# CWBudde/algo-dsp

Measured on AMD Instinct MI355X. Metric: Msamples/sec, overlap-save conv 131072-tap IR @48kHz; achieved HBM GB/s, higher is better.
Workload: dtype f64

## Files before the change

### algo-dsp_amd/csrc/conv_long_kernels.hip

```cpp
#include "conv_long_kernels.hpp"

#include "conv_kernels.hpp"
#include "fft_device.hpp"

namespace adsp {

constexpr int N1 = kLongN1, N2 = kLongN2, W = kLongW;
constexpr int kColThreads = 256;
constexpr int kRowsPerInstr = kColThreads / W;
constexpr int FS = N1 + 1;
using ColPlan = FftPlan<N1, 16>;
constexpr int RV = 8;
using RowPlan = FftPlan<N2, RV>;
static_assert(ColPlan::T * (W / 2) == kColThreads, "a tile's transforms fill the workgroup");
static_assert(N1 % kRowsPerInstr == 0, "whole load rounds");
static_assert(ColPlan::T <= 64 && 64 % ColPlan::T == 0, "a column transform sits inside one wave");

__global__ __launch_bounds__(kColThreads) void k_long_cols_fwd(LongColArgs a) {
  __shared__ double2 lds[(W / 2) * FS];
  __shared__ double2 ltab[TwSplit<N1>::N];
  const int tid = threadIdx.x;
  const int item = xcd_remap(blockIdx.x, gridDim.x);
  constexpr int kTiles = N2 / W;
  const int tile = item % kTiles, cb = item / kTiles;
  const int c = cb / a.blocks, j = cb % a.blocks;
  const int col = tid % W, r0 = tid / W;
  const int64_t b0 = a.start + (int64_t)j * a.hop + tile * W + col;
  const double* x = a.x + (int64_t)c * a.x_stride;
  double in[N1 / kRowsPerInstr];
#pragma unroll
  for (int i = 0; i < N1 / kRowsPerInstr; ++i) {
    const int64_t idx = b0 + (int64_t)(r0 + kRowsPerInstr * i) * N2;
    in[i] = (idx >= 0 && idx < a.n) ? x[idx] : 0.0;
  }
  const TwLds<N1> tw = tw_lds_compute<N1>(ltab, tid, kColThreads);
  double* img = reinterpret_cast<double*>(lds + (col >> 1) * FS) + (col & 1);
#pragma unroll
  for (int i = 0; i < N1 / kRowsPerInstr; ++i) img[2 * lds_slot(r0 + kRowsPerInstr * i)] = in[i];
  __syncthreads();
  const int f = tid / ColPlan::T, t = tid % ColPlan::T;
  double2* my = lds + f * FS;
  double2 v[16];
#pragma unroll
  for (int s = 0; s < 16; ++s) v[s] = my[pass0_slot<N1, 16>(t, s)];
  __syncthreads();
  fft_run<N1, 16, true>(v, t, my, tw);
  __syncthreads();
#pragma unroll
  for (int s = 0; s < 16; ++s) my[last_pass_slot<N1, 16>(t, s)] = v[s];
  __syncthreads();
  const double2* zc = lds + (col >> 1) * FS;
  double2* T = a.T + (int64_t)cb * kLongRows * kLongPitch + tile * W + col;
#pragma unroll
  for (int i = 0; i <= N1 / 2 / kRowsPerInstr; ++i) {
    const int k1 = r0 + kRowsPerInstr * i;
    if (k1 <= N1 / 2) {
      const double2 zk = zc[lds_slot(k1)];
      const double2 zm = zc[lds_slot((N1 - k1) & (N1 - 1))];
      const double2 o = (col & 1) ? make_double2(0.5 * (zk.y + zm.y), 0.5 * (zm.x - zk.x))
                                  : make_double2(0.5 * (zk.x + zm.x), 0.5 * (zk.y - zm.y));
      st2<true>(T + (int64_t)k1 * kLongPitch, o);
    }
  }
}

__global__ __launch_bounds__(kColThreads) void k_long_cols_inv(LongColArgs a) {
  __shared__ double2 lds[(W / 2) * FS];
  __shared__ double2 ltab[TwSplit<N1>::N];
  const int tid = threadIdx.x;
  const int item = xcd_remap(blockIdx.x, gridDim.x);
  constexpr int kTiles = N2 / W;
  const int tile = item % kTiles, cb = item / kTiles;
  const int c = cb / a.blocks, j = cb % a.blocks;
  const int col = tid % W, r0 = tid / W;
  const double2* T = a.T + (int64_t)cb * kLongRows * kLongPitch + tile * W + col;
  constexpr int NI = N1 / 2 / kRowsPerInstr + 1;
  double2 in[NI];
#pragma unroll
  for (int i = 0; i < NI; ++i) {
    const int k1 = r0 + kRowsPerInstr * i;
    in[i] = k1 <= N1 / 2 ? ld2<true>(T + (int64_t)k1 * kLongPitch) : make_double2(0, 0);
  }
  const TwLds<N1> tw = tw_lds_compute<N1>(ltab, tid, kColThreads);
  double2* zc = lds + (col >> 1) * FS;
#pragma unroll
  for (int i = 0; i < NI; ++i) {
    const int k1 = r0 + kRowsPerInstr * i;
    const double px = __shfl_xor(in[i].x, 1);
    const double py = __shfl_xor(in[i].y, 1);
    if (k1 <= N1 / 2) {
      if (!(col & 1)) {
        const bool edge = k1 == 0 || k1 == N1 / 2;
        zc[lds_slot(k1)] = edge ? make_double2(in[i].x, px) : make_double2(in[i].x - py, in[i].y + px);
      } else if (k1 != 0 && k1 != N1 / 2) {
        zc[lds_slot(N1 - k1)] = make_double2(px + in[i].y, in[i].x - py);
      }
    }
  }
  __syncthreads();
  const int f = tid / ColPlan::T, t = tid % ColPlan::T;
  double2* my = lds + f * FS;
  double2 v[16];
#pragma unroll
  for (int s = 0; s < 16; ++s) v[s] = my[pass0_slot<N1, 16>(t, s)];
  wave_lds_sync();
  fft_run_wave<N1, 16, false>(v, t, my, tw);
  wave_lds_sync();
#pragma unroll
  for (int s = 0; s < 16; ++s) my[last_pass_slot<N1, 16>(t, s)] = v[s];
  __syncthreads();
  const double* img = reinterpret_cast<const double*>(zc) + (col & 1);
  double* y = a.y + (int64_t)c * a.y_stride;
  const int64_t o0 = (int64_t)j * a.hop - a.skip + tile * W + col;
  const int64_t lo = (int64_t)j * a.hop;
  const int64_t hi = a.out_len < lo + a.hop ? a.out_len : lo + a.hop;
#pragma unroll
  for (int i = 0; i < N1 / kRowsPerInstr; ++i) {
    const int r = r0 + kRowsPerInstr * i;
    const int64_t o = o0 + (int64_t)r * N2;
    if (o >= lo && o < hi) y[o] = img[2 * lds_slot(r)];
  }
}

constexpr int kRowThreads = RowPlan::T;
static_assert(RowPlan::NPASS == 4 && RowPlan::R0 == RV && RV == 8 && kRowThreads == 8 * 64,
              "k_long_rows: four radix-8 passes over eight waves of 64 lanes, wave = k0");

__device__ __forceinline__ double wave_bcast(double x, int l) {
  const int lo = __builtin_amdgcn_readlane(__double2loint(x), l);
  const int hi = __builtin_amdgcn_readlane(__double2hiint(x), l);
  return __hiloint2double(hi, lo);
}

constexpr int kRowWavesPerSimd = 2 * kRowThreads / 256;
template <bool BUILD>
__global__ __launch_bounds__(kRowThreads, kRowWavesPerSimd) void k_long_rows(LongRowArgs a) {
  __shared__ double2 lds[N2];
  __shared__ double2 ltab[TwSplit<N2>::N];
  __shared__ double2 wtab[kRowThreads];
  constexpr int T = kRowThreads;
  const int tid = threadIdx.x;
  const int lane = tid & 63;
  const int wv = __builtin_amdgcn_readfirstlane(tid >> 6);
  const int l0 = lane & 7, l1 = lane & 56;
  const int item = xcd_remap(blockIdx.x, gridDim.x);
  const int ncb = a.blocks * a.channels;
  const int cb = item % ncb, k1 = item / ncb;
  double2* row = a.T + ((int64_t)cb * kLongRows + k1) * kLongPitch;
  double2 v[RV];
#pragma unroll
  for (int s = 0; s < RV; ++s) v[s] = ld2<true>(row + tid + T * s);
  const TwLds<N2> tw = tw_lds_compute<N2>(ltab, tid, T);
  double2 rt[RV];
  {
    double2 r;
    sincospi(-2.0 * (double)(T * k1 * l0) / (double)kLongN, &r.y, &r.x);
#pragma unroll
    for (int s = 0; s < RV; ++s) rt[s] = make_double2(wave_bcast(r.x, s), wave_bcast(r.y, s));
  }
  {
    double2 w0;
    sincospi(-2.0 * (double)(k1 * tid) / (double)kLongN, &w0.y, &w0.x);
    wtab[tid] = w0;
#pragma unroll
    for (int s = 0; s < RV; ++s) v[s] = c_mul(v[s], c_mul(w0, rt[s]));
  }
  Dft<RV, true>::run(v);
#pragma unroll
  for (int r = 0; r < RV; ++r) lds[T * r + tid] = v[r];
  double2 h[BUILD ? 1 : RV];
  if constexpr (!BUILD) {
    const double2* hrow = a.H + ((int64_t)a.ir_index[cb / a.blocks] * kLongRows + k1) * kLongPitch;
#pragma unroll
    for (int s = 0; s < RV; ++s) h[s] = hrow[tid + T * s];
  }
  __syncthreads();
  double2* sl = lds + 64 * RV * wv;
  double2 w = twiddle_root<N2, RV, 8, true>(wv, tw);
#pragma unroll
  for (int r = 0; r < RV; ++r) v[r] = sl[64 * r + lane];
  twiddle_powers<RV>(v, w);
  Dft<RV, true>::run(v);
  wave_lds_sync();
#pragma unroll
  for (int r = 0; r < RV; ++r) sl[8 * l1 + 8 * r + l0] = v[r];
  w = twiddle_root<N2, RV, 64, true>(l1 + wv, tw);
  wave_lds_sync();
#pragma unroll
  for (int r = 0; r < RV; ++r) v[r] = sl[64 * r + lane];
  twiddle_powers<RV>(v, w);
  Dft<RV, true>::run(v);
  wave_lds_sync();
#pragma unroll
  for (int r = 0; r < RV; ++r) sl[64 * l0 + ((l1 + r) ^ l0)] = v[r];
  w = twiddle_root<N2, RV, 512, true>(64 * l0 + l1 + wv, tw);
  wave_lds_sync();
#pragma unroll
  for (int r = 0; r < RV; ++r) v[r] = sl[64 * r + (lane ^ r)];
  twiddle_powers<RV>(v, w);
  Dft<RV, true>::run(v);
  if constexpr (BUILD) {
    double2* out = a.Hout + ((int64_t)cb * kLongRows + k1) * kLongPitch;
#pragma unroll
    for (int s = 0; s < RV; ++s) out[tid + T * s] = c_scale(v[s], a.scale);
  } else {
#pragma unroll
    for (int s = 0; s < RV; ++s) v[s] = c_mul(v[s], h[s]);
    Dft<RV, false>::run(v);
    wave_lds_sync();
#pragma unroll
    for (int r = 0; r < RV; ++r) sl[64 * l0 + ((l1 + r) ^ l0)] = v[r];
    w = twiddle_root<N2, RV, 8, false>(l0, tw);
    wave_lds_sync();
#pragma unroll
    for (int r = 0; r < RV; ++r) v[r] = sl[64 * r + (lane ^ r)];
    twiddle_powers<RV>(v, w);
    Dft<RV, false>::run(v);
    wave_lds_sync();
#pragma unroll
    for (int r = 0; r < RV; ++r) sl[8 * l1 + 8 * r + l0] = v[r];
    w = twiddle_root<N2, RV, 64, false>(lane, tw);
    wave_lds_sync();
#pragma unroll
    for (int r = 0; r < RV; ++r) v[r] = sl[64 * r + lane];
    twiddle_powers<RV>(v, w);
    Dft<RV, false>::run(v);
    wave_lds_sync();
#pragma unroll
    for (int r = 0; r < RV; ++r) sl[64 * r + lane] = v[r];
    w = twiddle_root<N2, RV, 512, false>(tid, tw);
    const double2 w0 = wtab[tid];
    __syncthreads();
#pragma unroll
    for (int r = 0; r < RV; ++r) v[r] = lds[T * r + tid];
    twiddle_powers<RV>(v, w);
    Dft<RV, false>::run(v);
#pragma unroll
    for (int s = 0; s < RV; ++s) st2<true>(row + tid + T * s, c_mul(v[s], c_conj(c_mul(w0, rt[s]))));
  }
}

void launch_long_cols_fwd(const LongColArgs& a, hipStream_t s) {
  const unsigned items = (unsigned)a.channels * a.blocks * (N2 / W);
  timed_launch(k_long_cols_fwd, dim3(items), dim3(kColThreads), s, a);
}

void launch_long_rows(const LongRowArgs& a, bool build_h, hipStream_t s) {
  const unsigned items = (unsigned)a.channels * a.blocks * kLongRows;
  if (build_h)
    timed_launch(k_long_rows<true>, dim3(items), dim3(kRowThreads), s, a);
  else
    timed_launch(k_long_rows<false>, dim3(items), dim3(kRowThreads), s, a);
}

void launch_long_cols_inv(const LongColArgs& a, hipStream_t s) {
  const unsigned items = (unsigned)a.channels * a.blocks * (N2 / W);
  timed_launch(k_long_cols_inv, dim3(items), dim3(kColThreads), s, a);
}

}
```

### algo-dsp_amd/csrc/conv_long_kernels.hpp

```cpp
#pragma once

#include <hip/hip_runtime.h>

#include <cstdint>

namespace adsp {

constexpr int kLongN1 = 512;
constexpr int kLongN2 = 4096;
constexpr int kLongW = 16;
constexpr int64_t kLongN = (int64_t)kLongN1 * kLongN2;
constexpr int kLongRows = kLongN1 / 2 + 1;
constexpr int kLongPitch = kLongN2 + 8;

struct LongColArgs {
  const double* x;
  int64_t x_stride, n, start, hop;
  int blocks, channels;
  double2* T;
  double* y;
  int64_t y_stride, out_len, skip;
};

struct LongRowArgs {
  double2* T;
  int blocks, channels;
  const double2* H;
  const int* ir_index;
  double2* Hout;
  double scale;
};

void launch_long_cols_fwd(const LongColArgs& a, hipStream_t s);
void launch_long_rows(const LongRowArgs& a, bool build_h, hipStream_t s);
void launch_long_cols_inv(const LongColArgs& a, hipStream_t s);

}
```

### algo-dsp_amd/csrc/fft_device.hpp

```cpp
#pragma once

#include <hip/hip_runtime.h>

namespace adsp {

struct cplx {
  double x, y;
};

typedef double d2v_t __attribute__((ext_vector_type(2)));
template <bool NT>
__device__ __forceinline__ double2 ld2(const double2* p) {
  if constexpr (NT) {
    const d2v_t t = __builtin_nontemporal_load(reinterpret_cast<const d2v_t*>(p));
    return make_double2(t.x, t.y);
  } else {
    return *p;
  }
}
template <bool NT>
__device__ __forceinline__ void st2(double2* p, double2 v) {
  if constexpr (NT)
    __builtin_nontemporal_store(d2v_t{v.x, v.y}, reinterpret_cast<d2v_t*>(p));
  else
    *p = v;
}

__device__ __forceinline__ double2 c_add(double2 a, double2 b) { return make_double2(a.x + b.x, a.y + b.y); }
__device__ __forceinline__ double2 c_sub(double2 a, double2 b) { return make_double2(a.x - b.x, a.y - b.y); }
__device__ __forceinline__ double2 c_mul(double2 a, double2 b) {
  return make_double2(a.x * b.x - a.y * b.y, a.x * b.y + a.y * b.x);
}
__device__ __forceinline__ double2 c_conj(double2 a) { return make_double2(a.x, -a.y); }
__device__ __forceinline__ double2 c_scale(double2 a, double s) { return make_double2(a.x * s, a.y * s); }

__device__ constexpr double kCos16[16] = {
    1.0,
    0.92387953251128675613,
    0.70710678118654752440,
    0.38268343236508977173,
    0.0,
    -0.38268343236508977173,
    -0.70710678118654752440,
    -0.92387953251128675613,
    -1.0,
    -0.92387953251128675613,
    -0.70710678118654752440,
    -0.38268343236508977173,
    0.0,
    0.38268343236508977173,
    0.70710678118654752440,
    0.92387953251128675613,
};

template <int E, bool FWD>
__device__ __forceinline__ double2 tw16(double2 a) {
  constexpr int e = E & 15;
  constexpr double R2 = 0.70710678118654752440;
  if constexpr (e == 0) {
    return a;
  } else if constexpr (e == 4) {
    return FWD ? make_double2(a.y, -a.x) : make_double2(-a.y, a.x);
  } else if constexpr (e == 8) {
    return make_double2(-a.x, -a.y);
  } else if constexpr (e == 12) {
    return FWD ? make_double2(-a.y, a.x) : make_double2(a.y, -a.x);
  } else if constexpr (e == 2) {
    return FWD ? make_double2((a.x + a.y) * R2, (a.y - a.x) * R2) : make_double2((a.x - a.y) * R2, (a.y + a.x) * R2);
  } else if constexpr (e == 6) {
    return FWD ? make_double2((a.y - a.x) * R2, -(a.x + a.y) * R2) : make_double2(-(a.x + a.y) * R2, (a.x - a.y) * R2);
  } else if constexpr (e == 10) {
    return FWD ? make_double2(-(a.x + a.y) * R2, (a.x - a.y) * R2) : make_double2((a.y - a.x) * R2, -(a.x + a.y) * R2);
  } else if constexpr (e == 14) {
    return FWD ? make_double2((a.x - a.y) * R2, (a.y + a.x) * R2) : make_double2((a.x + a.y) * R2, (a.y - a.x) * R2);
  } else {
    constexpr double c = kCos16[e];
    constexpr double s0 = kCos16[(e + 12) & 15];
    constexpr double s = FWD ? -s0 : s0;
    return make_double2(a.x * c - a.y * s, a.x * s + a.y * c);
  }
}

template <int R, bool FWD>
struct Dft {
  template <int I = 0>
  __device__ static __forceinline__ void combine(double2* v, const double2* e, const double2* o) {
    if constexpr (I < R / 2) {
      const double2 t = tw16<I*(16 / R), FWD>(o[I]);
      v[I] = c_add(e[I], t);
      v[I + R / 2] = c_sub(e[I], t);
      combine<I + 1>(v, e, o);
    }
  }
  __device__ static __forceinline__ void run(double2* v) {
    double2 e[R / 2], o[R / 2];
#pragma unroll
    for (int i = 0; i < R / 2; ++i) {
      e[i] = v[2 * i];
      o[i] = v[2 * i + 1];
    }
    Dft<R / 2, FWD>::run(e);
    Dft<R / 2, FWD>::run(o);
    combine(v, e, o);
  }
};
template <bool FWD>
struct Dft<1, FWD> {
  __device__ static __forceinline__ void run(double2*) {}
};

__host__ __device__ constexpr int ilog2c(int v) { return v <= 1 ? 0 : 1 + ilog2c(v >> 1); }
template <int M, int V = 16>
struct FftPlan {
  static_assert(M >= 16 && M <= 8192 && (M & (M - 1)) == 0, "FFT size must be a power of two in [16, 8192]");
  static_assert(V == 4 || V == 8 || V == 16, "4, 8 or 16 values per thread");
  static constexpr int LOGV = ilog2c(V);
  static constexpr int LOG = ilog2c(M);
  static constexpr int NPASS = (LOG + LOGV - 1) / LOGV;
  static constexpr int R0 = 1 << (LOG - LOGV * (NPASS - 1));
  static constexpr int T = M / V;
  static constexpr int BLOCK = T > 256 ? T : 256;
  static constexpr int F = BLOCK / T;
  static constexpr int MP = M + (T < 16 ? T : 0);
  static constexpr int radix(int p) { return p == 0 ? R0 : V; }
  static constexpr int ns(int p) { return p == 0 ? 1 : R0 * (1 << (LOGV * (p - 1))); }
};

__device__ __forceinline__ int xcd_remap(int b, int G) {
  const int xcd = b & 7, r = b >> 3;
  const int q = G >> 3, rem = G & 7;
  return (xcd < rem) ? xcd * (q + 1) + r : rem * (q + 1) + (xcd - rem) * q + r;
}

#ifndef AD_LDS_SWZ
#define AD_LDS_SWZ 1
#endif
__device__ __forceinline__ int lds_slot(int i) {
#if AD_LDS_SWZ
  const int t = (i >> 3) & 15;
  return i ^ (int)((0xde0321fc12cfed30ull >> (4 * t)) & 15);
#else
  const int q = i >> 4;
  return i ^ ((q ^ ((q & 4) << 1)) & 15);
#endif
}
__device__ __forceinline__ int lds_slot_split(int swz_base, int off) { return swz_base ^ lds_slot(off); }
__device__ __forceinline__ int tw_slot(int i) { return i ^ ((i >> 3) & 7); }

struct TwGlobal {
  const double2* __restrict__ t;
  __device__ __forceinline__ double2 operator()(int e) const { return t[e]; }
};
template <int M>
struct TwSplit {
  static constexpr int S = (ilog2c(M) + 1) / 2;
  static constexpr int NLO = 1 << S;
  static constexpr int NHI = M >> S;
  static constexpr int N = NLO + NHI;
};
template <int M>
struct TwLds {
  const double2* lo;
  const double2* hi;
  __device__ __forceinline__ double2 operator()(int e) const {
    using Sp = TwSplit<M>;
    if constexpr (Sp::NHI == 1) return lo[tw_slot(e)];
    const double2 a = lo[tw_slot(e & (Sp::NLO - 1))];
    const double2 b = hi[e >> Sp::S];
    return c_mul(a, b);
  }
};
template <int M, int STRIDE = 1>
__device__ __forceinline__ TwLds<M> tw_lds_fill(double2* ltab, const double2* __restrict__ g, int tid, int nthreads) {
  using Sp = TwSplit<M>;
  for (int i = tid; i < Sp::N; i += nthreads) {
    if (i < Sp::NLO)
      ltab[tw_slot(i)] = g[i * STRIDE];
    else
      ltab[i] = g[((i - Sp::NLO) << Sp::S) * STRIDE];
  }
  return TwLds<M>{ltab, ltab + Sp::NLO};
}

template <int M>
__device__ __forceinline__ TwLds<M> tw_lds_compute(double2* ltab, int tid, int nthreads) {
  using Sp = TwSplit<M>;
  for (int i = tid; i < Sp::N; i += nthreads) {
    const int e = i < Sp::NLO ? i : ((i - Sp::NLO) << Sp::S);
    double sn, cs;
    sincospi(-2.0 * (double)e / (double)M, &sn, &cs);
    ltab[i < Sp::NLO ? tw_slot(i) : i] = make_double2(cs, sn);
  }
  return TwLds<M>{ltab, ltab + Sp::NLO};
}

template <int M, int R, int NS, bool FWD, class TW>
__device__ __forceinline__ void apply_twiddles(double2* v, int jb, const TW& tw) {
  if constexpr (NS > 1) {
    const int e = (jb & (NS - 1)) * (M / (NS * R));
    double2 w = tw(e);
    if (!FWD) w = c_conj(w);
    double2 wr = w;
#pragma unroll
    for (int r = 1; r < R; ++r) {
      v[r] = c_mul(v[r], wr);
      if (r + 1 < R) wr = c_mul(wr, w);
    }
  }
}

template <int M, int V, int P, bool FWD, class TW>
__device__ __forceinline__ void pass_compute_store(double2* v, int tid, double2* lds, const TW& twM) {
  using Plan = FftPlan<M, V>;
  constexpr int R = Plan::radix(P);
  constexpr int NS = Plan::ns(P);
  constexpr int NB = V / R;
#pragma unroll
  for (int b = 0; b < NB; ++b) {
    const int jb = tid + b * Plan::T;
    apply_twiddles<M, R, NS, FWD, TW>(v + b * R, jb, twM);
    Dft<R, FWD>::run(v + b * R);
  }
#pragma unroll
  for (int b = 0; b < NB; ++b) {
    const int jb = tid + b * Plan::T;
    const int base = (jb / NS) * NS * R + (jb & (NS - 1));
    const int sb = lds_slot(base);
#pragma unroll
    for (int r = 0; r < R; ++r) lds[lds_slot_split(sb, r * NS)] = v[b * R + r];
  }
}

template <int M, int V, int P>
__device__ __forceinline__ void pass_load(double2* v, int tid, const double2* lds) {
  using Plan = FftPlan<M, V>;
  constexpr int R = Plan::radix(P);
  constexpr int NB = V / R;
#pragma unroll
  for (int b = 0; b < NB; ++b) {
    const int jb = tid + b * Plan::T;
    const int sb = lds_slot(jb);
#pragma unroll
    for (int r = 0; r < R; ++r) v[b * R + r] = lds[lds_slot_split(sb, r * (M / R))];
  }
}

template <int M, int V = 16>
__device__ __forceinline__ int pass0_index(int tid, int s) {
  using Plan = FftPlan<M, V>;
  constexpr int R = Plan::R0;
  const int b = s / R, r = s % R;
  return tid + b * Plan::T + r * (M / R);
}

template <int M, int V = 16>
__device__ __forceinline__ int pass0_slot(int tid, int s) {
  using Plan = FftPlan<M, V>;
  constexpr int R = Plan::R0;
  const int b = s / R, r = s % R;
  return lds_slot_split(lds_slot(tid + b * Plan::T), r * (M / R));
}

template <int M, int V, bool FWD, int P = 1, class TW>
__device__ __forceinline__ void run_middle_passes(double2* v, int tid, double2* lds, const TW& twM) {
  using Plan = FftPlan<M, V>;
  if constexpr (P < Plan::NPASS) {
    __syncthreads();
    pass_load<M, V, P>(v, tid, lds);
    if constexpr (P + 1 < Plan::NPASS) {
      __syncthreads();
      pass_compute_store<M, V, P, FWD, TW>(v, tid, lds, twM);
      run_middle_passes<M, V, FWD, P + 1, TW>(v, tid, lds, twM);
    }
  }
}

template <int M, int V, bool FWD, class TW>
__device__ __forceinline__ void last_pass_compute(double2* v, int tid, const TW& twM) {
  using Plan = FftPlan<M, V>;
  constexpr int P = Plan::NPASS - 1;
  constexpr int R = Plan::radix(P);
  constexpr int NS = Plan::ns(P);
  constexpr int NB = V / R;
#pragma unroll
  for (int b = 0; b < NB; ++b) {
    const int jb = tid + b * Plan::T;
    apply_twiddles<M, R, NS, FWD, TW>(v + b * R, jb, twM);
    Dft<R, FWD>::run(v + b * R);
  }
}

template <int M, int V = 16>
__device__ __forceinline__ int last_pass_index(int tid, int s) {
  using Plan = FftPlan<M, V>;
  constexpr int P = Plan::NPASS - 1;
  constexpr int R = Plan::radix(P);
  constexpr int NS = Plan::ns(P);
  const int b = s / R, r = s % R;
  const int jb = tid + b * Plan::T;
  return (jb / NS) * NS * R + (jb & (NS - 1)) + r * NS;
}

template <int M, int V = 16>
__device__ __forceinline__ int last_pass_slot(int tid, int s) {
  using Plan = FftPlan<M, V>;
  constexpr int P = Plan::NPASS - 1;
  constexpr int R = Plan::radix(P);
  constexpr int NS = Plan::ns(P);
  const int b = s / R, r = s % R;
  const int jb = tid + b * Plan::T;
  return lds_slot_split(lds_slot((jb / NS) * NS * R + (jb & (NS - 1))), r * NS);
}

template <int M, int V, bool FWD, class TW>
__device__ __forceinline__ void fft_run(double2* v, int tid, double2* lds, const TW& twM) {
  using Plan = FftPlan<M, V>;
  if constexpr (Plan::NPASS > 1) {
    pass_compute_store<M, V, 0, FWD, TW>(v, tid, lds, twM);
    run_middle_passes<M, V, FWD, 1, TW>(v, tid, lds, twM);
  }
  last_pass_compute<M, V, FWD, TW>(v, tid, twM);
}

__device__ __forceinline__ void wave_lds_sync() {
  __builtin_amdgcn_fence(__ATOMIC_RELEASE, "wavefront");
  __builtin_amdgcn_wave_barrier();
  __builtin_amdgcn_fence(__ATOMIC_ACQUIRE, "wavefront");
}

template <int M, int R, int NS, bool FWD, class TW>
__device__ __forceinline__ double2 twiddle_root(int jb, const TW& tw) {
  static_assert(NS > 1, "pass 0 has no twiddles");
  const double2 w = tw((jb & (NS - 1)) * (M / (NS * R)));
  return FWD ? w : c_conj(w);
}
template <int R>
__device__ __forceinline__ void twiddle_powers(double2* v, double2 w) {
  double2 wr = w;
#pragma unroll
  for (int r = 1; r < R; ++r) {
    v[r] = c_mul(v[r], wr);
    if (r + 1 < R) wr = c_mul(wr, w);
  }
}

template <int M, int V, bool FWD, int P = 1, class TW>
__device__ __forceinline__ void run_middle_passes_wave(double2* v, int tid, double2* lds, const TW& twM) {
  using Plan = FftPlan<M, V>;
  if constexpr (P < Plan::NPASS) {
    wave_lds_sync();
    pass_load<M, V, P>(v, tid, lds);
    if constexpr (P + 1 < Plan::NPASS) {
      wave_lds_sync();
      pass_compute_store<M, V, P, FWD, TW>(v, tid, lds, twM);
      run_middle_passes_wave<M, V, FWD, P + 1, TW>(v, tid, lds, twM);
    }
  }
}
template <int M, int V, bool FWD, class TW>
__device__ __forceinline__ void fft_run_wave(double2* v, int tid, double2* lds, const TW& twM) {
  using Plan = FftPlan<M, V>;
  static_assert(Plan::T <= 64 && 64 % Plan::T == 0, "the transform's threads must sit inside one wave");
  if constexpr (Plan::NPASS > 1) {
    pass_compute_store<M, V, 0, FWD, TW>(v, tid, lds, twM);
    run_middle_passes_wave<M, V, FWD, 1, TW>(v, tid, lds, twM);
  }
  last_pass_compute<M, V, FWD, TW>(v, tid, twM);
}

template <int M, int V, bool FWD, int P = 1, class TW>
__device__ __forceinline__ void run_middle_passes_active(double2* v, int tid, double2* lds, const TW& twM, bool active) {
  using Plan = FftPlan<M, V>;
  if constexpr (P < Plan::NPASS) {
    __syncthreads();
    if (active) pass_load<M, V, P>(v, tid, lds);
    if constexpr (P + 1 < Plan::NPASS) {
      __syncthreads();
      if (active) pass_compute_store<M, V, P, FWD, TW>(v, tid, lds, twM);
      run_middle_passes_active<M, V, FWD, P + 1, TW>(v, tid, lds, twM, active);
    }
  }
}
template <int M, int V, bool FWD, class TW>
__device__ __forceinline__ void fft_run_active(double2* v, int tid, double2* lds, const TW& twM, bool active) {
  using Plan = FftPlan<M, V>;
  if constexpr (Plan::NPASS > 1) {
    if (active) pass_compute_store<M, V, 0, FWD, TW>(v, tid, lds, twM);
    run_middle_passes_active<M, V, FWD, 1, TW>(v, tid, lds, twM, active);
  }
  if (active) last_pass_compute<M, V, FWD, TW>(v, tid, twM);
}

}
```

Baseline: 89190.

## Precompute tile bounds and split LDS swizzle to cut per-element address math in column kernels

Column forward and inverse kernels now classify each row group of a tile as fully inside, straddling, or outside the valid range once per tile. They use 32-bit offsets and unguarded loads and stores for the inside groups, so the 64-bit index math and per-element bounds checks go away. LDS swizzle addresses are split into a per-thread base plus a compile-time part, and the mirror-index reads are batched. The lane shuffle is replaced with a DPP quad permute. Together these reduce VALU and address overhead but add intricate boundary logic that could mis-handle edge tiles.

```diff
diff --git a/algo-dsp_amd/csrc/conv_long_kernels.hip b/algo-dsp_amd/csrc/conv_long_kernels.hip
--- a/algo-dsp_amd/csrc/conv_long_kernels.hip
+++ b/algo-dsp_amd/csrc/conv_long_kernels.hip
@@ -16,6 +16,19 @@
 static_assert(N1 % kRowsPerInstr == 0, "whole load rounds");
 static_assert(ColPlan::T <= 64 && 64 % ColPlan::T == 0, "a column transform sits inside one wave");
 
+static_assert(kRowsPerInstr == 16 && kRowsPerInstr == kLongTileRows, "lds_slot_split16: r0 is the low nibble of the row");
+static_assert(N1 / 2 % kRowsPerInstr == 0, "row N1/2 is instruction N1/2 / kRowsPerInstr of r0 = 0");
+constexpr int kHalfInstr = N1 / 2 / kRowsPerInstr;
+
+__device__ __forceinline__ int mirror_slot(int sm, int r0, int i) {
+  constexpr int kTop = N1 / kRowsPerInstr - 1;
+  const int h = kTop - i, k = h & 7;
+  const int base = r0 ? (sm ^ (lds_slot(kRowsPerInstr * k) & 15))
+                      : kRowsPerInstr + (lds_slot(kRowsPerInstr * ((k + 1) & 7)) & 15);
+  if (i == 0) return r0 ? kRowsPerInstr * h + base : 0;
+  return kRowsPerInstr * h + base;
+}
+
 __global__ __launch_bounds__(kColThreads) void k_long_cols_fwd(LongColArgs a) {
   __shared__ double2 lds[(W / 2) * FS];
   __shared__ double2 ltab[TwSplit<N1>::N];
@@ -25,18 +38,31 @@
   const int tile = item % kTiles, cb = item / kTiles;
   const int c = cb / a.blocks, j = cb % a.blocks;
   const int col = tid % W, r0 = tid / W;
-  const int64_t b0 = a.start + (int64_t)j * a.hop + tile * W + col;
-  const double* x = a.x + (int64_t)c * a.x_stride;
+  const int64_t origin = a.start + (int64_t)j * a.hop;
+  const LongBlockRange rng = long_block_range(origin, 0, a.n);
+  const LongTileBounds tb = long_tile_bounds(tile, rng);
+  const double* x = a.x + (int64_t)c * a.x_stride + origin;
+  const unsigned xoff = r0 * N2 + col;
   double in[N1 / kRowsPerInstr];
 #pragma unroll
   for (int i = 0; i < N1 / kRowsPerInstr; ++i) {
-    const int64_t idx = b0 + (int64_t)(r0 + kRowsPerInstr * i) * N2;
-    in[i] = (idx >= 0 && idx < a.n) ? x[idx] : 0.0;
+    const int first = long_tile_first(tile, i);
+    if (long_tile_inside(i, tb)) {
+      in[i] = (x + first)[xoff];
+    } else if (long_tile_touched(i, tb)) {
+      const int e = first + (int)xoff;
+      const bool ok = long_point_valid(e, rng);
+      const double xe = x[ok ? e : rng.lo];
+      in[i] = ok ? xe : 0.0;
+    } else {
+      in[i] = 0.0;
+    }
   }
   const TwLds<N1> tw = tw_lds_compute<N1>(ltab, tid, kColThreads);
   double* img = reinterpret_cast<double*>(lds + (col >> 1) * FS) + (col & 1);
-#pragma unroll
-  for (int i = 0; i < N1 / kRowsPerInstr; ++i) img[2 * lds_slot(r0 + kRowsPerInstr * i)] = in[i];
+  const int sk = lds_slot(r0);
+#pragma unroll
+  for (int i = 0; i < N1 / kRowsPerInstr; ++i) img[2 * lds_slot_split16(sk, kRowsPerInstr * i)] = in[i];
   __syncthreads();
   const int f = tid / ColPlan::T, t = tid % ColPlan::T;
   double2* my = lds + f * FS;
@@ -50,17 +76,30 @@
   for (int s = 0; s < 16; ++s) my[last_pass_slot<N1, 16>(t, s)] = v[s];
   __syncthreads();
   const double2* zc = lds + (col >> 1) * FS;
-  double2* T = a.T + (int64_t)cb * kLongRows * kLongPitch + tile * W + col;
-#pragma unroll
-  for (int i = 0; i <= N1 / 2 / kRowsPerInstr; ++i) {
-    const int k1 = r0 + kRowsPerInstr * i;
-    if (k1 <= N1 / 2) {
-      const double2 zk = zc[lds_slot(k1)];
-      const double2 zm = zc[lds_slot((N1 - k1) & (N1 - 1))];
-      const double2 o = (col & 1) ? make_double2(0.5 * (zk.y + zm.y), 0.5 * (zm.x - zk.x))
-                                  : make_double2(0.5 * (zk.x + zm.x), 0.5 * (zk.y - zm.y));
-      st2<true>(T + (int64_t)k1 * kLongPitch, o);
+  const int sm = lds_slot((kRowsPerInstr - r0) & (kRowsPerInstr - 1));
+  double2* T = a.T + (int64_t)cb * kLongRows * kLongPitch + tile * W;
+  const unsigned toff = r0 * kLongPitch + col;
+  const auto separate = [col](double2 zk, double2 zm) {
+    return (col & 1) ? make_double2(0.5 * (zk.y + zm.y), 0.5 * (zm.x - zk.x))
+                     : make_double2(0.5 * (zk.x + zm.x), 0.5 * (zk.y - zm.y));
+  };
+  constexpr int kBatch = 8;
+  static_assert(kHalfInstr % kBatch == 0, "whole batches");
+#pragma unroll
+  for (int b = 0; b < kHalfInstr; b += kBatch) {
+    double2 zk[kBatch], zm[kBatch];
+#pragma unroll
+    for (int u = 0; u < kBatch; ++u) {
+      zk[u] = zc[lds_slot_split16(sk, kRowsPerInstr * (b + u))];
+      zm[u] = zc[mirror_slot(sm, r0, b + u)];
     }
+#pragma unroll
+    for (int u = 0; u < kBatch; ++u)
+      st2<true>(T + (int64_t)(b + u) * kRowsPerInstr * kLongPitch + toff, separate(zk[u], zm[u]));
+  }
+  if (r0 == 0) {
+    const double2 zh = zc[lds_slot(N1 / 2)];
+    st2<true>(T + (int64_t)(N1 / 2) * kLongPitch + toff, separate(zh, zh));
   }
 }
 
@@ -73,28 +112,29 @@
   const int tile = item % kTiles, cb = item / kTiles;
   const int c = cb / a.blocks, j = cb % a.blocks;
   const int col = tid % W, r0 = tid / W;
-  const double2* T = a.T + (int64_t)cb * kLongRows * kLongPitch + tile * W + col;
-  constexpr int NI = N1 / 2 / kRowsPerInstr + 1;
-  double2 in[NI];
-#pragma unroll
-  for (int i = 0; i < NI; ++i) {
-    const int k1 = r0 + kRowsPerInstr * i;
-    in[i] = k1 <= N1 / 2 ? ld2<true>(T + (int64_t)k1 * kLongPitch) : make_double2(0, 0);
-  }
+  const double2* T = a.T + (int64_t)cb * kLongRows * kLongPitch + tile * W;
+  const unsigned toff = r0 * kLongPitch + col;
+  double2 in[kHalfInstr + 1];
+#pragma unroll
+  for (int i = 0; i < kHalfInstr; ++i) in[i] = ld2<true>(T + (int64_t)i * kRowsPerInstr * kLongPitch + toff);
+  in[kHalfInstr] = r0 == 0 ? ld2<true>(T + (int64_t)(N1 / 2) * kLongPitch + toff) : make_double2(0, 0);
   const TwLds<N1> tw = tw_lds_compute<N1>(ltab, tid, kColThreads);
   double2* zc = lds + (col >> 1) * FS;
-#pragma unroll
-  for (int i = 0; i < NI; ++i) {
-    const int k1 = r0 + kRowsPerInstr * i;
-    const double px = __shfl_xor(in[i].x, 1);
-    const double py = __shfl_xor(in[i].y, 1);
-    if (k1 <= N1 / 2) {
-      if (!(col & 1)) {
-        const bool edge = k1 == 0 || k1 == N1 / 2;
-        zc[lds_slot(k1)] = edge ? make_double2(in[i].x, px) : make_double2(in[i].x - py, in[i].y + px);
-      } else if (k1 != 0 && k1 != N1 / 2) {
-        zc[lds_slot(N1 - k1)] = make_double2(px + in[i].y, in[i].x - py);
-      }
+  const int sk = lds_slot(r0);
+  const int sm = lds_slot((kRowsPerInstr - r0) & (kRowsPerInstr - 1));
+  const bool even = !(col & 1);
+#pragma unroll
+  for (int i = 0; i <= kHalfInstr; ++i) {
+    const double px = lane_xor1(in[i].x);
+    const double py = lane_xor1(in[i].y);
+    if (i == kHalfInstr) {
+      if (even && r0 == 0) zc[lds_slot(N1 / 2)] = make_double2(in[i].x, px);
+    } else if (even) {
+      const bool edge = i == 0 && r0 == 0;
+      zc[lds_slot_split16(sk, kRowsPerInstr * i)] =
+          edge ? make_double2(in[i].x, px) : make_double2(in[i].x - py, in[i].y + px);
+    } else if (i != 0 || r0 != 0) {
+      zc[mirror_slot(sm, r0, i)] = make_double2(px + in[i].y, in[i].x - py);
     }
   }
   __syncthreads();
@@ -111,14 +151,25 @@
   __syncthreads();
   const double* img = reinterpret_cast<const double*>(zc) + (col & 1);
   double* y = a.y + (int64_t)c * a.y_stride;
-  const int64_t o0 = (int64_t)j * a.hop - a.skip + tile * W + col;
   const int64_t lo = (int64_t)j * a.hop;
   const int64_t hi = a.out_len < lo + a.hop ? a.out_len : lo + a.hop;
-#pragma unroll
-  for (int i = 0; i < N1 / kRowsPerInstr; ++i) {
-    const int r = r0 + kRowsPerInstr * i;
-    const int64_t o = o0 + (int64_t)r * N2;
-    if (o >= lo && o < hi) y[o] = img[2 * lds_slot(r)];
+  const int64_t origin = lo - a.skip;
+  const LongBlockRange rng = long_block_range(origin, lo, hi);
+  const LongTileBounds tb = long_tile_bounds(tile, rng);
+  y += origin;
+  const unsigned yoff = r0 * N2 + col;
+  double out[N1 / kRowsPerInstr];
+#pragma unroll
+  for (int i = 0; i < N1 / kRowsPerInstr; ++i)
+    if (long_tile_inside(i, tb)) out[i] = img[2 * lds_slot_split16(sk, kRowsPerInstr * i)];
+#pragma unroll
+  for (int i = 0; i < N1 / kRowsPerInstr; ++i)
+    if (long_tile_inside(i, tb)) (y + long_tile_first(tile, i))[yoff] = out[i];
+#pragma unroll 1
+  for (int i = long_tile_next_straddling(tb.any_first - 1, tb); i < tb.any_first + tb.any_count;
+       i = long_tile_next_straddling(i, tb)) {
+    const int first = long_tile_first(tile, i);
+    if (long_point_valid(first + (int)yoff, rng)) (y + first)[yoff] = img[2 * lds_slot(r0 + kRowsPerInstr * i)];
   }
 }
 
diff --git a/algo-dsp_amd/csrc/conv_long_kernels.hpp b/algo-dsp_amd/csrc/conv_long_kernels.hpp
--- a/algo-dsp_amd/csrc/conv_long_kernels.hpp
+++ b/algo-dsp_amd/csrc/conv_long_kernels.hpp
@@ -12,6 +12,57 @@
 constexpr int64_t kLongN = (int64_t)kLongN1 * kLongN2;
 constexpr int kLongRows = kLongN1 / 2 + 1;
 constexpr int kLongPitch = kLongN2 + 8;
+
+constexpr int kLongTileRows = 256 / kLongW;
+constexpr int kLongTileStepLog2 = 16;
+constexpr int kLongTileStep = kLongTileRows * kLongN2;
+constexpr int kLongTileSpan = (kLongTileRows - 1) * kLongN2 + kLongW - 1;
+static_assert(kLongTileStep == 1 << kLongTileStepLog2, "long_tile_bounds divides by shifting");
+struct LongBlockRange {
+  int lo, hi;
+};
+__host__ __device__ constexpr LongBlockRange long_block_range(int64_t origin, int64_t lo, int64_t hi) {
+  const int64_t a = lo - origin, b = hi - origin;
+  const int l = (int)(a < 0 ? 0 : a > kLongN ? kLongN : a);
+  const int h = (int)(b < 0 ? 0 : b > kLongN ? kLongN : b);
+  return h > l ? LongBlockRange{l, h} : LongBlockRange{0, 0};
+}
+__host__ __device__ constexpr bool long_point_valid(int e, LongBlockRange r) {
+  return (unsigned)(e - r.lo) < (unsigned)(r.hi - r.lo);
+}
+struct LongTileBounds {
+  int in_first, in_count, any_first, any_count;
+};
+__host__ __device__ constexpr LongTileBounds long_tile_bounds(int tile, LongBlockRange r) {
+  const int t = tile * kLongW;
+  const int in_first = (r.lo - t + kLongTileStep - 1) >> kLongTileStepLog2;
+  const int in_last = (r.hi - 1 - kLongTileSpan - t) >> kLongTileStepLog2;
+  const int any_first = (r.lo - kLongTileSpan - t + kLongTileStep - 1) >> kLongTileStepLog2;
+  const int any_last = (r.hi - 1 - t) >> kLongTileStepLog2;
+  const int in_count = in_last - in_first + 1, any_count = any_last - any_first + 1;
+  return {in_first, in_count > 0 ? in_count : 0, any_first, any_count > 0 ? any_count : 0};
+}
+__host__ __device__ constexpr bool long_tile_inside(int i, LongTileBounds b) {
+  return (unsigned)(i - b.in_first) < (unsigned)b.in_count;
+}
+__host__ __device__ constexpr bool long_tile_touched(int i, LongTileBounds b) {
+  return (unsigned)(i - b.any_first) < (unsigned)b.any_count;
+}
+__host__ __device__ constexpr int long_tile_next_straddling(int i, LongTileBounds b) {
+  ++i;
+  return b.in_count > 0 && i == b.in_first ? i + b.in_count : i;
+}
+enum LongTileClass : int { kLongTileInside = 0, kLongTileOutside = 1, kLongTileStraddle = 2 };
+__host__ __device__ constexpr LongTileClass long_tile_class(int i, LongTileBounds b) {
+  return long_tile_inside(i, b) ? kLongTileInside : long_tile_touched(i, b) ? kLongTileStraddle : kLongTileOutside;
+}
+__host__ __device__ constexpr int long_tile_first(int tile, int i) { return tile * kLongW + i * kLongTileStep; }
+static_assert(long_tile_class(1, long_tile_bounds(kLongN2 / kLongW - 1, long_block_range(-131071, 0, kLongN - 131071))) ==
+                      kLongTileStraddle &&
+                  long_tile_class(1, long_tile_bounds(kLongN2 / kLongW - 2, long_block_range(-131071, 0, kLongN - 131071))) ==
+                      kLongTileOutside &&
+                  long_tile_class(2, long_tile_bounds(0, long_block_range(-131071, 0, kLongN - 131071))) == kLongTileInside,
+              "tile bounds at the bench's own skip");
 
 struct LongColArgs {
   const double* x;
diff --git a/algo-dsp_amd/csrc/fft_device.hpp b/algo-dsp_amd/csrc/fft_device.hpp
--- a/algo-dsp_amd/csrc/fft_device.hpp
+++ b/algo-dsp_amd/csrc/fft_device.hpp
@@ -145,6 +145,16 @@
 #endif
 }
 __device__ __forceinline__ int lds_slot_split(int swz_base, int off) { return swz_base ^ lds_slot(off); }
+__device__ __forceinline__ int lds_slot_split16(int swz_base, int off16) {
+  return off16 + (swz_base ^ (lds_slot(off16) & 15));
+}
+
+__device__ __forceinline__ double lane_xor1(double x) {
+  constexpr int kQuadPerm1032 = 1 | (0 << 2) | (3 << 4) | (2 << 6);
+  const int lo = __builtin_amdgcn_mov_dpp(__double2loint(x), kQuadPerm1032, 0xf, 0xf, true);
+  const int hi = __builtin_amdgcn_mov_dpp(__double2hiint(x), kQuadPerm1032, 0xf, 0xf, true);
+  return __hiloint2double(hi, lo);
+}
 __device__ __forceinline__ int tw_slot(int i) { return i ^ ((i >> 3) & 7); }
 
 struct TwGlobal {
```

After: 90720 (median of 6 runs). +1.7%, better.
